# andrewcsmith/soundsym

Hardware: AMD Instinct MI355X
Metric: segment-pairs/sec (DTW cost+argmin) (higher is better)
Workload: dtype f32

## Files before the change

### soundsym_amd/csrc/dtw_filter_kernel.hpp

```cpp
#pragma once
#include <hip/hip_runtime.h>

#ifndef SSYM_FILTER_MODE
#define SSYM_FILTER_MODE 0
#endif

namespace ssym {

typedef _Float16 half8 __attribute__((ext_vector_type(8)));
typedef float f32x16 __attribute__((ext_vector_type(16)));

constexpr int kFilterRowsPerTile = 16;
constexpr int kFilterKM = 3;
constexpr int kFilterRecHalfs = 48;
constexpr int kFilterMaxDim2 = 13;
constexpr int kFilterMaxDim1 = 42;

__host__ __device__ constexpr int filter_slot_offset(int k) { return ((k >> 3) & 1) * 24 + (k >> 4) * 8 + (k & 7); }

template <int KM>
__device__ __forceinline__ f32x16 mfma_tile(const half8 (&a)[KM], const half8 (&b)[KM])
{
    f32x16 acc = {0, 0, 0, 0, 0, 0, 0, 0, 0, 0, 0, 0, 0, 0, 0, 0};
#if SSYM_FILTER_MODE == 2
    float z = (float)a[0][0] + (float)b[0][0];
    asm volatile("" : "+v"(z));
#pragma unroll
    for (int r = 0; r < 16; ++r)
        acc[r] = z + (float)r;
    return acc;
#else
#ifndef SSYM_ABL_DROP_MFMA
#define SSYM_ABL_DROP_MFMA 0
#endif
#pragma unroll
    for (int m = 0; m < KM - SSYM_ABL_DROP_MFMA; ++m)
        acc = __builtin_amdgcn_mfma_f32_32x32x16_f16(a[m], b[m], acc, 0, 0, 0);
    return acc;
#endif
}

template <int KU>
__device__ __forceinline__ void load_rec(const _Float16 *__restrict__ p, half8 (&dst)[KU])
{
#pragma unroll
    for (int m = 0; m < KU; ++m)
        dst[m] = *reinterpret_cast<const half8 *>(p + 8 * m);
}

constexpr int kTgtFrameHalfs = kFilterKM * 512;
__host__ __device__ constexpr size_t tgt_rec_offset(uint32_t t, uint32_t slots, uint32_t j, int m, int h)
{
    return (((size_t)(t >> 5) * slots + j) * kFilterKM + m) * 512 + (size_t)(h * 32 + (t & 31u)) * 8;
}
template <int KU>
__device__ __forceinline__ void load_tgt_rec(const _Float16 *__restrict__ p, int j, half8 (&dst)[KU])
{
#pragma unroll
    for (int m = 0; m < KU; ++m)
        dst[m] = *reinterpret_cast<const half8 *>(p + (size_t)j * kTgtFrameHalfs + m * 512);
}

template <int NT, bool SQ, int KU, bool SKIP0 = false>
__device__ __forceinline__ float dp_column(const half8 (&A)[NT][KU], const half8 (&Bc)[KU],
                                           const half8 (&Bn)[KU], f32x16 &acc, float up, float diag,
                                           const float (&Lr)[NT * 16], float (&Lw)[NT * 16], const bool skip0 = false)
{
#pragma unroll
    for (int T = 0; T < NT; ++T) {
        f32x16 accn;
        if (T + 1 < NT)
            accn = mfma_tile<KU>(A[T + 1], Bc);
        else
            accn = mfma_tile<KU>(A[0], Bn);
#if SSYM_FILTER_MODE == 1
        asm volatile("" ::"v"(acc[0]), "v"(acc[15]));
        up = acc[3];
        Lw[T * 16] = Lr[T * 16];
#else
        if (SKIP0 && T == 0 && skip0) {
            up = __builtin_inff();
            diag = __builtin_inff();
        } else {
#pragma unroll
            for (int r = 0; r < 16; ++r) {
                const int idx = T * 16 + r;
                const float x = acc[r];
                const float c = SQ ? __builtin_fabsf(x) : __builtin_amdgcn_sqrtf(__builtin_fabsf(x));
                const float m = __builtin_fminf(__builtin_fminf(up, diag), Lr[idx]);
                diag = Lr[idx];
                const float cur = c + m;
                Lw[idx] = cur;
                up = cur;
            }
        }
#endif
        acc = accn;
    }
    return up;
}

constexpr int kFilterWavesPerBlock = 4;

#define SSYM_FILTER_SBASE(P_) asm volatile("" : "+s"(P_))
#define SSYM_FILTER_LANEOFF(V_) asm volatile("" : "+v"(V_))
#ifndef SSYM_PRUNE_EVERY
#define SSYM_PRUNE_EVERY 8
#endif
#ifndef SSYM_PRUNE_FINE
#define SSYM_PRUNE_FINE 48
#endif
constexpr int kPruneFine = SSYM_PRUNE_FINE;
constexpr int kPruneEvery = SSYM_PRUNE_EVERY;
constexpr int kTaskCtrStride = 64;
constexpr int filter_ring(int occ) { return occ >= 3 ? 2 : 4; }
constexpr int kFilterSlotBytes = kFilterKM * 1024;
constexpr int kFilterTopBytes = 2 * 1024;
constexpr int filter_wave_lds(int occ) { return filter_ring(occ) * kFilterSlotBytes + kFilterTopBytes; }
constexpr int wait_vmcnt(int n) { return 0x0F70 | (n & 15) | ((n >> 4) << 14); }

template <int NT, bool SQ, int OCC = 2, bool PRUNE = false, int KU = kFilterKM, bool SKIP0 = false>
__global__ __launch_bounds__(64 * kFilterWavesPerBlock, OCC) void dtw_filter_kernel(
    const _Float16 *__restrict__ srcRec, const _Float16 *__restrict__ tgtRec,
    const int *__restrict__ srcLen, const int *__restrict__ tgtLen, int srcRows, int nPasses,
    int tgtFramesPad, int mPad, int nSrcPairs, int nTasks, int taskChunk, float outScale,
    float *__restrict__ handoff, unsigned *__restrict__ taskCtr, float *__restrict__ cmat,
    const float *__restrict__ abandon = nullptr, unsigned long long *__restrict__ colCtr = nullptr,
    const uint32_t *__restrict__ candSlot = nullptr, int rowOrigin = 0, int spBase = 0)
{
    static_assert(!SKIP0 || (!PRUNE && NT >= 2), "SKIP0: unpruned launches of at least two tiles");
    constexpr int REC = kFilterRecHalfs;
    constexpr int BR = NT * 16;
    const float INF = __builtin_inff();

    const int lane = threadIdx.x & 63;
    const int wave = __builtin_amdgcn_readfirstlane(threadIdx.x >> 6);
    const int col = lane & 31;
    const int half = lane >> 5;
    const size_t handGroups = ((size_t)tgtFramesPad + 3) / 4;
    char *const handRow = reinterpret_cast<char *>(handoff + ((size_t)blockIdx.x * kFilterWavesPerBlock + wave) * handGroups * 256);
    uint32_t laneOff16 = lane * 16;
    const __amdgpu_buffer_rsrc_t handBuf = __builtin_amdgcn_make_buffer_rsrc(handRow, 0, (int)(handGroups * 1024), 0x00020000);
    constexpr int kFilterRing = filter_ring(OCC);
    constexpr int kWaitLead = wait_vmcnt(KU * (kFilterRing - 2)), kWaitFirst = wait_vmcnt(KU * (kFilterRing - 1));
    __shared__ __attribute__((aligned(16))) char ring[kFilterWavesPerBlock][filter_wave_lds(OCC)];
    char *const myRing = ring[wave];
    char *const myTop = myRing + kFilterRing * kFilterSlotBytes;

    unsigned colSteps = 0;
    const unsigned nGroups = (unsigned)mPad >> 5;
    for (unsigned hop = 0; hop < 8; ++hop) {
      const unsigned xcd = (blockIdx.x + hop) & 7u;
      const unsigned rangeLen = xcd < nGroups ? ((nGroups - xcd + 7u) >> 3) * (unsigned)nSrcPairs : 0u;
      for (;;) {
        unsigned got = 0;
        if (lane == 0)
            got = atomicAdd(&taskCtr[xcd * kTaskCtrStride], (unsigned)taskChunk);
        got = (unsigned)__builtin_amdgcn_readfirstlane((int)got);
        if (got >= rangeLen)
            break;
        const unsigned gotEnd = min(got + (unsigned)taskChunk, rangeLen);
        int preFa = 0, preFb = 0;
        bool havePre = false;
       for (unsigned gi = got; gi < gotEnd; ++gi) {
        const unsigned lin = rangeLen - 1u - gi;
        const int tg = (int)(xcd + 8u * (lin / (unsigned)nSrcPairs));
        const int sp = spBase + (int)(lin % (unsigned)nSrcPairs);

        const int fa = havePre ? preFa : srcLen[2 * sp + half];
        const int fb_m1 = (havePre ? preFb : tgtLen[32 * tg + col]) - 1;
        havePre = gi + 1 < gotEnd;
        if (havePre) {
            const unsigned linN = lin - 1u;
            preFa = srcLen[2 * (spBase + (int)(linN % (unsigned)nSrcPairs)) + half];
            preFb = tgtLen[32 * (int)(xcd + 8u * (linN / (unsigned)nSrcPairs)) + col];
        }
        const int r0 = srcRows - fa;

        int nCols = fb_m1 + 1, r0min = r0;
#pragma unroll
        for (int o = 32; o >= 1; o >>= 1) {
            nCols = max(nCols, __shfl_xor(nCols, o));
            r0min = min(r0min, __shfl_xor(r0min, o));
        }
        nCols = __builtin_amdgcn_readfirstlane(nCols);
        r0min = __builtin_amdgcn_readfirstlane(r0min);
        const int firstPass = min(max(r0min - rowOrigin, 0) / BR, nPasses - 1);

        float res = INF;
        float thr = INF;
        bool dropped = false;
        int lastTop = -1;
        if (PRUNE)
            thr = abandon[32 * tg + col];
        bool dead = fa == 0 || fb_m1 < 0;
        if (PRUNE)
            dead = dead || candSlot[32 * tg + col] == (uint32_t)(2 * sp + half);
        const char *const tgtGroup = reinterpret_cast<const char *>(tgtRec) + (size_t)tg * tgtFramesPad * (kTgtFrameHalfs * 2);

        for (int pass = nCols > 0 ? firstPass : nPasses; pass < nPasses && !dropped; ++pass) {
            const int rowBase = rowOrigin + pass * BR;
#ifdef SSYM_ABL_NOHAND
            const bool haveTop = false;
#else
            const bool haveTop = pass > firstPass;
#endif
            const bool lastPass = pass == nPasses - 1;
            const bool skip0 = SKIP0 && r0min - rowBase >= 17;
            const bool started = r0 < rowBase + BR;

            auto stage = [&](int c) {
                const int cc = min(c, nCols - 1);
                char *slot = myRing + (c & (kFilterRing - 1)) * kFilterSlotBytes;
                const char *gb = tgtGroup + (size_t)(unsigned)cc * (kTgtFrameHalfs * 2);
                static_assert(KU == 2 || KU == 3, "two or three operand planes per column");
                SSYM_FILTER_SBASE(gb);
                SSYM_FILTER_LANEOFF(laneOff16);
                const __attribute__((address_space(1))) void *gp =
                    (const __attribute__((address_space(1))) void *)(gb + laneOff16);
                __attribute__((address_space(3))) void *lp = (__attribute__((address_space(3))) void *)slot;
                __builtin_amdgcn_global_load_lds(gp, lp, 16, 0, 0);
                __builtin_amdgcn_global_load_lds(gp, lp, 16, 1024, 0);
                if (KU == 3)
                    __builtin_amdgcn_global_load_lds(gp, lp, 16, 2048, 0);
            };
            auto stageTop = [&](int g) {
                const int gg = min(g, (nCols - 1) >> 2);
                __builtin_amdgcn_raw_ptr_buffer_load_lds(handBuf, (__attribute__((address_space(3))) void *)(myTop + (g & 1) * 1024),
                                                         16, laneOff16, gg * 1024, 0, 0);
            };
            auto fetch = [&](int c, half8 (&B)[KU], float &top) {
                const char *slot = myRing + (c & (kFilterRing - 1)) * kFilterSlotBytes;
#pragma unroll
                for (int m = 0; m < KU; ++m)
                    B[m] = *reinterpret_cast<const half8 *>(slot + m * 1024 + lane * 16);
                top = *reinterpret_cast<const float *>(myTop + ((c >> 2) & 1) * 1024 + (c & 3) * 256 + lane * 4);
            };
            half8 A[NT][KU];
            {
                const int arow = lane & 31;
                const int a_src = 2 * sp + ((arow >> 2) & 1);
                const int a_frm = rowBase + (arow & 3) + 4 * (arow >> 3);
                const _Float16 *abase = srcRec + ((size_t)a_src * srcRows + a_frm) * REC + half * 24;
#pragma unroll
                for (int T = 0; T < NT; ++T)
                    load_rec<KU>(abase + (size_t)T * kFilterRowsPerTile * REC, A[T]);
            }

            asm volatile("" ::: "memory");
            if (haveTop)
                stageTop(0);
#pragma unroll
            for (int c = 0; c < kFilterRing; ++c)
                stage(c);

            float L0[BR], L1[BR];
#pragma unroll
            for (int i = 0; i < BR; ++i) {
                L0[i] = (rowBase + i == r0 - 1) ? 0.0f : INF;
                L1[i] = L0[i];
            }
            float prevTop = (rowBase == r0) ? 0.0f : INF;

            half8 B0[KU], B1[KU];
            float topN = INF;
            __builtin_amdgcn_s_waitcnt(kWaitFirst);
            asm volatile("" ::: "memory");
            if (!PRUNE && !haveTop) {
                typedef float f32x4 __attribute__((ext_vector_type(4)));
                *reinterpret_cast<f32x4 *>(myTop + lane * 16) = f32x4{INF, INF, INF, INF};
                *reinterpret_cast<f32x4 *>(myTop + 1024 + lane * 16) = f32x4{INF, INF, INF, INF};
            }
            fetch(0, B0, topN);
            f32x16 acc = mfma_tile<KU>(A[0], B0);

            float runBot = INF;
            bool passOver = false;
            int lastCol = nCols - 1;
            for (int j0 = 0; j0 < nCols && !passOver; j0 += 4) {
                if (PRUNE)
                    colSteps += (unsigned)min(4, nCols - j0);
#pragma unroll
                for (int q = 0; q < 4; ++q) {
                    const int j = j0 + q;
                    if (j < nCols) {
                        const float up = (!PRUNE || (haveTop && j <= lastTop)) ? topN : INF;
                        const float diag = prevTop;
                        prevTop = up;
                        __builtin_amdgcn_s_waitcnt(kWaitLead);
                        asm volatile("" ::: "memory");
                        if ((q & 1) == 0)
                            fetch(j + 1, B1, topN);
                        else
                            fetch(j + 1, B0, topN);
#ifndef SSYM_ABL_NOSTAGE
                        stage(j + kFilterRing);
#endif
                        if (q == 0 && haveTop)
                            stageTop((j >> 2) + 1);
                        float bottom;
                        if ((q & 1) == 0)
                            bottom = dp_column<NT, SQ, KU, SKIP0>(A, B0, B1, acc, up, diag, L0, L1, skip0);
                        else
                            bottom = dp_column<NT, SQ, KU, SKIP0>(A, B1, B0, acc, up, diag, L1, L0, skip0);
                        if (!lastPass) {
#ifndef SSYM_ABL_NOHAND
                            __builtin_amdgcn_raw_buffer_store_b32(__float_as_uint(bottom), handBuf, lane * 4, (j >> 2) * 1024 + q * 256, 0);
#else
                            res = (j == fb_m1 - 1) ? bottom : res;
#endif
                        } else {
                            res = (j == fb_m1) ? bottom : res;
                        }
                        if (PRUNE) {
                            runBot = __builtin_fminf(runBot, bottom);
                            if (q == 3 && (j < kPruneFine || (j & (kPruneEvery - 1)) == kPruneEvery - 1)) {
                                float cm = L0[0];
#pragma unroll
                                for (int i = 1; i < BR; i += 2)
                                    cm = __builtin_fminf(__builtin_fminf(cm, L0[i]), i + 1 < BR ? L0[i + 1] : L0[i]);
                                const bool quiet = !(cm <= thr) || j >= fb_m1 || dead;
                                if (__all(quiet) && j >= lastTop) {
                                    passOver = true;
                                    lastCol = j;
                                }
                            }
                        }
                    }
                }
            }
            if (PRUNE && !lastPass) {
                lastTop = lastCol;
                dropped = __all((started && !(runBot <= thr)) || dead);
            }
        }
        cmat[(size_t)(2 * sp + half) * mPad + 32 * tg + col] = res * outScale;
       }
      }
    }
    if (PRUNE && colCtr && lane == 0)
        atomicAdd(colCtr, (unsigned long long)colSteps * BR);
}

#undef SSYM_FILTER_SBASE
#undef SSYM_FILTER_LANEOFF

}
```

Measured before the change: 507.4 million.

## Specialize DTW row passes by kind and unroll columns by eight

For unpruned launches with small tile counts, the row-pass body becomes a lambda instantiated per pass kind: not-last, last-uniform and last-ragged. Each instance drops the per-column branches on lastPass and on the result select. The handoff store of the bottom cell is deferred by one column and read from the L array, so it is off the dp_column critical path. Uniform last passes read the result once at the end, and the column loop is unrolled by eight with compile-time ring and top phases. The cost is larger code, more register pressure and more complex handoff indexing.

```diff
diff --git a/soundsym_amd/csrc/dtw_filter_kernel.hpp b/soundsym_amd/csrc/dtw_filter_kernel.hpp
--- a/soundsym_amd/csrc/dtw_filter_kernel.hpp
+++ b/soundsym_amd/csrc/dtw_filter_kernel.hpp
@@ -101,6 +101,8 @@
 }
 
 constexpr int kFilterWavesPerBlock = 4;
+enum : int { kPassNotLast = 0, kPassLastRagged = 1, kPassLastUniform = 2, kPassAny = 3 };
+template <int K> struct PassKind { static constexpr int value = K; };
 
 #define SSYM_FILTER_SBASE(P_) asm volatile("" : "+s"(P_))
 #define SSYM_FILTER_LANEOFF(V_) asm volatile("" : "+v"(V_))
@@ -131,6 +133,8 @@
     static_assert(!SKIP0 || (!PRUNE && NT >= 2), "SKIP0: unpruned launches of at least two tiles");
     constexpr int REC = kFilterRecHalfs;
     constexpr int BR = NT * 16;
+    constexpr bool SPLIT = !PRUNE && NT <= 4;
+    constexpr int CU = SPLIT ? 8 : 4;
     const float INF = __builtin_inff();
 
     const int lane = threadIdx.x & 63;
@@ -187,6 +191,7 @@
         r0min = __builtin_amdgcn_readfirstlane(r0min);
         const int firstPass = min(max(r0min - rowOrigin, 0) / BR, nPasses - 1);
 
+        const bool uniform = SPLIT && __all(fb_m1 == nCols - 1 && fa != 0);
         float res = INF;
         float thr = INF;
         bool dropped = false;
@@ -229,106 +234,132 @@
                 __builtin_amdgcn_raw_ptr_buffer_load_lds(handBuf, (__attribute__((address_space(3))) void *)(myTop + (g & 1) * 1024),
                                                          16, laneOff16, gg * 1024, 0, 0);
             };
-            auto fetch = [&](int c, half8 (&B)[KU], float &top) {
-                const char *slot = myRing + (c & (kFilterRing - 1)) * kFilterSlotBytes;
+            auto fetch = [&](int c, int ph, half8 (&B)[KU], float &top) {
+                const char *slot = myRing + (ph & (kFilterRing - 1)) * kFilterSlotBytes;
 #pragma unroll
                 for (int m = 0; m < KU; ++m)
                     B[m] = *reinterpret_cast<const half8 *>(slot + m * 1024 + lane * 16);
-                top = *reinterpret_cast<const float *>(myTop + ((c >> 2) & 1) * 1024 + (c & 3) * 256 + lane * 4);
+                const int ct = CU % 8 == 0 ? ph : c;
+                top = *reinterpret_cast<const float *>(myTop + ((ct >> 2) & 1) * 1024 + (ct & 3) * 256 + lane * 4);
             };
-            half8 A[NT][KU];
-            {
-                const int arow = lane & 31;
-                const int a_src = 2 * sp + ((arow >> 2) & 1);
-                const int a_frm = rowBase + (arow & 3) + 4 * (arow >> 3);
-                const _Float16 *abase = srcRec + ((size_t)a_src * srcRows + a_frm) * REC + half * 24;
-#pragma unroll
-                for (int T = 0; T < NT; ++T)
-                    load_rec<KU>(abase + (size_t)T * kFilterRowsPerTile * REC, A[T]);
-            }
-
-            asm volatile("" ::: "memory");
-            if (haveTop)
-                stageTop(0);
-#pragma unroll
-            for (int c = 0; c < kFilterRing; ++c)
-                stage(c);
-
-            float L0[BR], L1[BR];
-#pragma unroll
-            for (int i = 0; i < BR; ++i) {
-                L0[i] = (rowBase + i == r0 - 1) ? 0.0f : INF;
-                L1[i] = L0[i];
-            }
-            float prevTop = (rowBase == r0) ? 0.0f : INF;
-
-            half8 B0[KU], B1[KU];
-            float topN = INF;
-            __builtin_amdgcn_s_waitcnt(kWaitFirst);
-            asm volatile("" ::: "memory");
-            if (!PRUNE && !haveTop) {
-                typedef float f32x4 __attribute__((ext_vector_type(4)));
-                *reinterpret_cast<f32x4 *>(myTop + lane * 16) = f32x4{INF, INF, INF, INF};
-                *reinterpret_cast<f32x4 *>(myTop + 1024 + lane * 16) = f32x4{INF, INF, INF, INF};
-            }
-            fetch(0, B0, topN);
-            f32x16 acc = mfma_tile<KU>(A[0], B0);
-
             float runBot = INF;
             bool passOver = false;
             int lastCol = nCols - 1;
-            for (int j0 = 0; j0 < nCols && !passOver; j0 += 4) {
-                if (PRUNE)
-                    colSteps += (unsigned)min(4, nCols - j0);
-#pragma unroll
-                for (int q = 0; q < 4; ++q) {
-                    const int j = j0 + q;
-                    if (j < nCols) {
-                        const float up = (!PRUNE || (haveTop && j <= lastTop)) ? topN : INF;
-                        const float diag = prevTop;
-                        prevTop = up;
-                        __builtin_amdgcn_s_waitcnt(kWaitLead);
-                        asm volatile("" ::: "memory");
-                        if ((q & 1) == 0)
-                            fetch(j + 1, B1, topN);
-                        else
-                            fetch(j + 1, B0, topN);
+            auto rowPass = [&](auto kindTag) __attribute__((always_inline)) {
+                constexpr int KIND = decltype(kindTag)::value;
+                half8 A[NT][KU];
+                {
+                    const int arow = lane & 31;
+                    const int a_src = 2 * sp + ((arow >> 2) & 1);
+                    const int a_frm = rowBase + (arow & 3) + 4 * (arow >> 3);
+                    const _Float16 *abase = srcRec + ((size_t)a_src * srcRows + a_frm) * REC + half * 24;
+#pragma unroll
+                    for (int T = 0; T < NT; ++T)
+                        load_rec<KU>(abase + (size_t)T * kFilterRowsPerTile * REC, A[T]);
+                }
+
+                asm volatile("" ::: "memory");
+                if (haveTop)
+                    stageTop(0);
+#pragma unroll
+                for (int c = 0; c < kFilterRing; ++c)
+                    stage(c);
+
+                float L0[BR], L1[BR];
+#pragma unroll
+                for (int i = 0; i < BR; ++i) {
+                    L0[i] = (rowBase + i == r0 - 1) ? 0.0f : INF;
+                    L1[i] = L0[i];
+                }
+                float prevTop = (rowBase == r0) ? 0.0f : INF;
+
+                half8 B0[KU], B1[KU];
+                float topN = INF;
+                __builtin_amdgcn_s_waitcnt(kWaitFirst);
+                asm volatile("" ::: "memory");
+                if (!PRUNE && !haveTop) {
+                    typedef float f32x4 __attribute__((ext_vector_type(4)));
+                    *reinterpret_cast<f32x4 *>(myTop + lane * 16) = f32x4{INF, INF, INF, INF};
+                    *reinterpret_cast<f32x4 *>(myTop + 1024 + lane * 16) = f32x4{INF, INF, INF, INF};
+                }
+                fetch(0, 0, B0, topN);
+                f32x16 acc = mfma_tile<KU>(A[0], B0);
+
+                for (int j0 = 0; j0 < nCols && !passOver; j0 += CU) {
+#pragma unroll
+                    for (int q = 0; q < CU; ++q) {
+                        const int j = j0 + q;
+                        if (j < nCols) {
+                            if (PRUNE && (q & 3) == 0)
+                                colSteps += (unsigned)min(4, nCols - j);
+                            const float up = (!PRUNE || (haveTop && j <= lastTop)) ? topN : INF;
+                            const float diag = prevTop;
+                            prevTop = up;
+                            __builtin_amdgcn_s_waitcnt(kWaitLead);
+                            asm volatile("" ::: "memory");
+                            if ((q & 1) == 0)
+                                fetch(j + 1, (q + 1) & (CU - 1), B1, topN);
+                            else
+                                fetch(j + 1, (q + 1) & (CU - 1), B0, topN);
+#ifndef SSYM_ABL_NOHAND
+                            if (KIND == kPassNotLast && (q > 0 || j0 > 0))
+                                __builtin_amdgcn_raw_buffer_store_b32(__float_as_uint((q & 1) == 0 ? L0[BR - 1] : L1[BR - 1]), handBuf,
+                                                                      lane * 4, (j - 1) * 256, 0);
+#endif
 #ifndef SSYM_ABL_NOSTAGE
-                        stage(j + kFilterRing);
-#endif
-                        if (q == 0 && haveTop)
-                            stageTop((j >> 2) + 1);
-                        float bottom;
-                        if ((q & 1) == 0)
-                            bottom = dp_column<NT, SQ, KU, SKIP0>(A, B0, B1, acc, up, diag, L0, L1, skip0);
-                        else
-                            bottom = dp_column<NT, SQ, KU, SKIP0>(A, B1, B0, acc, up, diag, L1, L0, skip0);
-                        if (!lastPass) {
-#ifndef SSYM_ABL_NOHAND
-                            __builtin_amdgcn_raw_buffer_store_b32(__float_as_uint(bottom), handBuf, lane * 4, (j >> 2) * 1024 + q * 256, 0);
+                            stage(j + kFilterRing);
+#endif
+                            if ((q & 3) == 0 && haveTop)
+                                stageTop((j >> 2) + 1);
+                            float bottom;
+                            if ((q & 1) == 0)
+                                bottom = dp_column<NT, SQ, KU, SKIP0>(A, B0, B1, acc, up, diag, L0, L1, skip0);
+                            else
+                                bottom = dp_column<NT, SQ, KU, SKIP0>(A, B1, B0, acc, up, diag, L1, L0, skip0);
+                            if (KIND == kPassNotLast || (KIND == kPassAny && !lastPass)) {
+#ifdef SSYM_ABL_NOHAND
+                                res = (j == fb_m1 - 1) ? bottom : res;
 #else
-                            res = (j == fb_m1 - 1) ? bottom : res;
-#endif
-                        } else {
-                            res = (j == fb_m1) ? bottom : res;
-                        }
-                        if (PRUNE) {
-                            runBot = __builtin_fminf(runBot, bottom);
-                            if (q == 3 && (j < kPruneFine || (j & (kPruneEvery - 1)) == kPruneEvery - 1)) {
-                                float cm = L0[0];
-#pragma unroll
-                                for (int i = 1; i < BR; i += 2)
-                                    cm = __builtin_fminf(__builtin_fminf(cm, L0[i]), i + 1 < BR ? L0[i + 1] : L0[i]);
-                                const bool quiet = !(cm <= thr) || j >= fb_m1 || dead;
-                                if (__all(quiet) && j >= lastTop) {
-                                    passOver = true;
-                                    lastCol = j;
+                                if (KIND == kPassAny)
+                                    __builtin_amdgcn_raw_buffer_store_b32(__float_as_uint(bottom), handBuf, lane * 4, j * 256, 0);
+#endif
+                            } else if (KIND == kPassLastRagged || KIND == kPassAny) {
+                                res = (j == fb_m1) ? bottom : res;
+                            }
+                            if (PRUNE) {
+                                runBot = __builtin_fminf(runBot, bottom);
+                                if ((q & 3) == 3 && (j < kPruneFine || (j & (kPruneEvery - 1)) == kPruneEvery - 1)) {
+                                    float cm = L0[0];
+#pragma unroll
+                                    for (int i = 1; i < BR; i += 2)
+                                        cm = __builtin_fminf(__builtin_fminf(cm, L0[i]), i + 1 < BR ? L0[i + 1] : L0[i]);
+                                    const bool quiet = !(cm <= thr) || j >= fb_m1 || dead;
+                                    if (__all(quiet) && j >= lastTop) {
+                                        passOver = true;
+                                        lastCol = j;
+                                    }
                                 }
                             }
                         }
                     }
                 }
-            }
+#ifndef SSYM_ABL_NOHAND
+                if (KIND == kPassNotLast) {
+                    const int jl = nCols - 1;
+                    __builtin_amdgcn_raw_buffer_store_b32(__float_as_uint((jl & 1) ? L0[BR - 1] : L1[BR - 1]), handBuf, lane * 4, jl * 256, 0);
+                }
+#endif
+                if (KIND == kPassLastUniform)
+                    res = ((nCols - 1) & 1) ? L0[BR - 1] : L1[BR - 1];
+            };
+            if (!SPLIT)
+                rowPass(PassKind<kPassAny>{});
+            else if (!lastPass)
+                rowPass(PassKind<kPassNotLast>{});
+            else if (uniform)
+                rowPass(PassKind<kPassLastUniform>{});
+            else
+                rowPass(PassKind<kPassLastRagged>{});
             if (PRUNE && !lastPass) {
                 lastTop = lastCol;
                 dropped = __all((started && !(runBot <= thr)) || dead);
```

Result: no change. 508.1 million, median of 2 (+0.1%).
